# MycroftAI/mycroft-precise

Hardware: AMD Instinct MI355X
Metric: MFCC+GRU windows/sec (node); max concurrent real-time 16 kHz streams (higher is better)
Workload: dtype f32

## Files before the change

### include/precise_engine.h

```cpp
#ifndef PRECISE_ENGINE_H
#define PRECISE_ENGINE_H

#include <stddef.h>
#include <stdint.h>

#ifdef __cplusplus
extern "C" {
#endif

#define PE_ABI_VERSION 8

typedef enum pe_status {
    PE_OK = 0,
    PE_ERR_INVALID = 1,
    PE_ERR_HIP = 2,
    PE_ERR_UNSUPPORTED = 3,
    PE_ERR_NOMEM = 4,
    PE_ERR_EOF = 5
} pe_status;

typedef struct pe_params {
    int32_t sample_rate;
    int32_t window_samples;
    int32_t hop_samples;
// ... 100 lines not shown
int pe_get_info(const pe_engine* e, pe_info* out);

int pe_get_stream_state(pe_engine* e, int32_t* q_out, uint32_t* computed_out, uint32_t* emitted_out);

int pe_set_renumber_at(pe_engine* e, uint32_t call_number);

int pe_set_fused(pe_engine* e, int32_t enabled);

int pe_set_input_projection(pe_engine* e, int32_t enabled);

int pe_set_gru_waves(pe_engine* e, int32_t waves_per_tile);

int pe_set_gru_tiling(pe_engine* e, int32_t tiling);
int pe_get_gru_tiling(const pe_engine* e);

int pe_set_timing(pe_engine* e, int32_t enabled);
int pe_get_last_timing(pe_engine* e, float* mfcc_ms, float* gru_ms);

#ifdef __cplusplus
}
#endif
#endif
```

### mycroft_precise_amd/_lib.py

```python
import ctypes as C
import importlib.util
import os
import weakref

import numpy as np

HERE = os.path.dirname(os.path.abspath(__file__))
LIB_PATH = os.environ.get('PE_LIB') or os.path.join(HERE, 'libprecise_engine.so')

PE_OK, PE_ERR_INVALID, PE_ERR_HIP, PE_ERR_UNSUPPORTED, PE_ERR_NOMEM, PE_ERR_EOF = range(6)
ABI_VERSION = 8


class PeParams(C.Structure):
    _fields_ = [(n, C.c_int32) for n in (
        'sample_rate', 'window_samples', 'hop_samples', 'n_fft', 'n_filt', 'n_mfcc', 'n_features',
        'use_delta', 'mfcc_precision', 'gru_precision', 'vectorizer', 'ring_precision')]


class PeGruLayer(C.Structure):
    _fields_ = [('n_in', C.c_int32), ('units', C.c_int32),
                ('kernel', C.POINTER(C.c_float)), ('recurrent_kernel', C.POINTER(C.c_float)),
                ('bias', C.POINTER(C.c_float))]

# ... 46 lines not shown
                                   C.POINTER(C.c_int64)]),
    'pe_evaluate': (C.c_int, [C.c_void_p, C.c_void_p, C.c_int64, C.c_int32, C.c_void_p, C.c_int64,
                              C.POINTER(C.c_int64)]),
    'pe_set_decoder': (C.c_int, [C.c_void_p, C.c_void_p, C.c_int32, C.c_int32, C.c_int32, C.c_double]),
    'pe_set_trigger': (C.c_int, [C.c_void_p, C.c_int32, C.c_double, C.c_int32]),
    'pe_set_decoder_model': (C.c_int, [C.c_void_p, C.c_int32, C.c_void_p, C.c_int32, C.c_int32, C.c_int32, C.c_double]),
    'pe_set_trigger_model': (C.c_int, [C.c_void_p, C.c_int32, C.c_int32, C.c_double, C.c_int32]),
    'pe_decode_device': (C.c_int, [C.c_void_p, C.c_void_p, C.c_void_p, C.c_void_p, C.c_void_p]),
    'pe_decode': (C.c_int, [C.c_void_p, C.c_void_p, C.c_void_p, C.c_void_p]),
    'pe_get_info': (C.c_int, [C.c_void_p, C.POINTER(PeInfo)]),
    'pe_get_stream_state': (C.c_int, [C.c_void_p, C.c_void_p, C.c_void_p, C.c_void_p]),
    'pe_set_fused': (C.c_int, [C.c_void_p, C.c_int32]),
    'pe_set_gru_waves': (C.c_int, [C.c_void_p, C.c_int32]),
    'pe_set_gru_tiling': (C.c_int, [C.c_void_p, C.c_int32]),
    'pe_get_gru_tiling': (C.c_int, [C.c_void_p]),
    'pe_set_input_projection': (C.c_int, [C.c_void_p, C.c_int32]),
    'pe_set_timing': (C.c_int, [C.c_void_p, C.c_int32]),
    'pe_get_last_timing': (C.c_int, [C.c_void_p, C.POINTER(C.c_float), C.POINTER(C.c_float)]),
}

_lib = None


class HipLibraryMissing(ImportError):
    pass


def _preload_hip_runtime():
    if os.environ.get('PRECISE_AMD_HIP_RUNTIME', '') == 'system':
        return
# ... 305 lines not shown
    def info(self) -> PeInfo:
        i = PeInfo()
        self._check(self._lib.pe_get_info(self._h, C.byref(i)))
        return i

    def stream_state(self):
        q = np.empty(self.n_streams, dtype=np.int32)
        kc = np.empty(self.n_streams, dtype=np.uint32)
        ke = np.empty(self.n_streams, dtype=np.uint32)
        self._check(self._lib.pe_get_stream_state(self._h, q.ctypes.data, kc.ctypes.data, ke.ctypes.data))
        return q, kc, ke

    def set_fused(self, enabled: bool):
        self._check(self._lib.pe_set_fused(self._h, int(bool(enabled))))

    def set_input_projection(self, enabled: bool):
        self._check(self._lib.pe_set_input_projection(self._h, int(bool(enabled))))

    def set_gru_waves(self, waves: int):
        self._check(self._lib.pe_set_gru_waves(self._h, int(waves)))

    def set_gru_tiling(self, tiling: int):
        self._check(self._lib.pe_set_gru_tiling(self._h, int(tiling)))

    def gru_tiling(self) -> int:
        return int(self._lib.pe_get_gru_tiling(self._h))

    def set_timing(self, enabled: bool):
        self._check(self._lib.pe_set_timing(self._h, int(bool(enabled))))

# ... 23 lines not shown
```

### mycroft_precise_amd/csrc/engine.hip

```cpp
#include "../../include/precise_engine.h"
#include "pe_common.h"
#include "gru_cw_pack.h"
#include "mfcc_general_device.h"

#include <algorithm>
#include <cmath>
#include <cstdarg>
#include <cstdio>
#include <cstdlib>
#include <cstring>
#include <string>
#include <vector>

using namespace pe;

namespace {

thread_local std::string g_global_error;

struct DeviceBuf {
    void* p = nullptr;
    size_t bytes = 0;
};

// ... 28 lines not shown
    int64_t device_bytes = 0;
    StreamRec* rec = nullptr;
    int16_t* carry = nullptr;
    const int16_t* kept = nullptr; int kept_chunk = 0;
    const int16_t* call_head = nullptr; int call_head_chunk = 0; bool call_keep = false;
    uint32_t call_no = 1;
    uint32_t renumber_at = 0x7fff0000u;
    bool fused = true;
    int gru_waves = 0;
    bool general = false;
    int row_floats = kRowFloats;
    int carry_cap = kCarryCap;
    GeneralTables gtab{};
    int gru_tiling = -1;
    float* cw_blob = nullptr;
    int n_cus = 256;
    float* ring = nullptr;
    float* proj_ring = nullptr;
    bool proj_ok = false, proj_on = false;
    std::vector<float> proj_w_host, proj_b_host;
    int max_updates = 1;
    uint32_t* ke_hist = nullptr;
    unsigned char* table_blob = nullptr;
    pe_wave::Layout table_layout{};
    float* wxd = nullptr;
    float* wx = nullptr; float* wr1 = nullptr; float* wr2 = nullptr; float* bias = nullptr; float* wd = nullptr;
    bool wide = false;
    float* wide_buf[2][6] = {{nullptr}};
    int wide_kx4[2] = {1, 1};
    float* wide_wd = nullptr;
// ... 735 lines not shown
    for (int m = 0; m < e->n_models; ++m) {
        GruArgs gm = with_model(e, g, m);
        gm.out = g.out + (size_t)m * (size_t)out_stride;
        const int rc = launch_network(e, gm, mode, s, m);
        if (rc) return rc;
    }
    return PE_OK;
}
int launch_networks_many(pe_engine* e, const GruArgs& g, int n_updates, hipStream_t s) {
    if (e->n_models == 1) { PE_HIP(e, launch_gru_many(g, n_updates, e->n_padded, s)); return PE_OK; }
    const ModelSet ms = model_set(e, g);
    PE_HIP(e, launch_gru_many(g, n_updates, e->n_padded, s, &ms, e->n_models));
    return PE_OK;
}

int launch_gru_ring(pe_engine* e, float* out_dev, hipStream_t s, const int32_t* ids = nullptr, int n_active = 0) {
    GruArgs a = gru_args(e);
    a.out = out_dev;
    if (ids) { a.ids = ids; a.n_streams = n_active; }
    return launch_networks(e, a, 1, s, a.n_streams);
}

bool is_pinned(const pe_engine* e, const void* p, size_t bytes) {
    const char* c = static_cast<const char*>(p);
    for (const auto& r : e->pinned)
        if (c >= r.first && c + bytes <= r.first + r.second) return true;
    return false;
}

int async_init(pe_engine* e) {
    if (e->s_compute) return PE_OK;
    PE_HIP(e, hipStreamCreateWithFlags(&e->s_copy, hipStreamNonBlocking));
// ... 86 lines not shown
    }
    if (!keep_call && (rc = flush_kept(e, s))) return rc;
    e->call_head = keep_call ? e->kept : nullptr; e->call_head_chunk = e->kept_chunk; e->call_keep = keep_call;
    struct Reset { pe_engine* e; ~Reset() { e->call_head = nullptr; e->call_head_chunk = 0; e->call_keep = false; } } reset{e};
    e->kept = keep_call ? pcm_dev : nullptr; e->kept_chunk = keep_call ? chunk : 0;
    uint32_t call = 0;
    if ((rc = begin_state_call(e, s, &call))) return rc;
    if (t) { PE_HIP(e, hipEventRecord(e->ev[0], s)); }
    if (raw_out_dev && can_fuse(e, chunk)) {
        GruArgs g = gru_args(e);
        g.call = call;
        g.predict_ke = 1;
        g.chunk = chunk;
        g.out = raw_out_dev;
        if (ids) { g.ids = ids; g.n_streams = n_active; }
        if (e->n_models > 1) {
            const ModelSet ms = model_set(e, g);
            if (e->prm.mfcc_precision == 0) PE_HIP(e, launch_fused_models_f64(mfcc_args<double>(e, pcm_dev, chunk, call, ids, n_active), tables<double>(e), g, ms, e->n_models, e->n_cus, s));
            else PE_HIP(e, launch_fused_models_f32(mfcc_args<float>(e, pcm_dev, chunk, call, ids, n_active), tables<float>(e), g, ms, e->n_models, e->n_cus, s));
        }
        else if (e->prm.mfcc_precision == 0) PE_HIP(e, launch_fused_f64(mfcc_args<double>(e, pcm_dev, chunk, call, ids, n_active), tables<double>(e), g, e->n_cus, s));
        else PE_HIP(e, launch_fused_f32(mfcc_args<float>(e, pcm_dev, chunk, call, ids, n_active), tables<float>(e), g, e->n_cus, s));
        if (t) { PE_HIP(e, hipEventRecord(e->ev[1], s)); PE_HIP(e, hipEventRecord(e->ev[2], s)); e->ev_valid = true; e->ev_has_gru = false; }
    } else {
        if ((rc = launch_mfcc(e, pcm_dev, chunk, s, call, ids, n_active))) return rc;
        if (t) { PE_HIP(e, hipEventRecord(e->ev[1], s)); }
        if (raw_out_dev) {
            if ((rc = launch_gru_ring(e, raw_out_dev, s, ids, n_active))) return rc;
        }
        if (t) { PE_HIP(e, hipEventRecord(e->ev[2], s)); e->ev_valid = true; e->ev_has_gru = raw_out_dev != nullptr; }
    }
    if (feats_out_dev) {
        GatherArgs g{e->n_streams, e->prm.n_features, e->prm.n_mfcc, e->ring_slots, e->prm.ring_precision, e->ring, state_of(e, e->call_no + 1u), feats_out_dev, e->row_floats};
        PE_HIP(e, launch_gather(g, s));
    }
    return PE_OK;
}

}

extern "C" {

int pe_abi_version(void) { return PE_ABI_VERSION; }
// ... 223 lines not shown
    PE_HIP(e, hipSetDevice(e->device));
    PE_DRAIN(e);
    const uint8_t* mask_dev = nullptr;
    if (mask_host) {
        int rc = ensure(e, e->st_mask, (size_t)e->n_streams);
        if (rc) return rc;
        PE_HIP(e, hipMemcpy(e->st_mask.p, mask_host, (size_t)e->n_streams, hipMemcpyHostToDevice));
        mask_dev = static_cast<const uint8_t*>(e->st_mask.p);
    }
    if (mask_dev) { int frc = flush_kept(e, nullptr); if (frc) return frc; }
    else { e->kept = nullptr; e->kept_chunk = 0; }
    uint32_t call = 0;
    { int crc = begin_state_call(e, nullptr, &call); if (crc) return crc; }
    ClearArgs a{e->n_padded, e->ring_slots, mask_dev, state_of(e, call), e->ring, e->prm.ring_precision, e->activation,
                e->proj_on ? e->proj_ring : nullptr,
                e->proj_on ? reinterpret_cast<const float*>(e->table_blob + e->table_layout.proj_b) : nullptr, e->row_floats};
    if (mask_dev) a.n_streams = e->n_streams;
    PE_HIP(e, launch_clear(a, nullptr));
    if (e->n_models > 1 && e->activation)
        PE_HIP(e, launch_clear_activation(mask_dev, e->activation, a.n_streams, e->n_padded, e->n_models - 1, nullptr));
    PE_HIP(e, hipStreamSynchronize(nullptr));
    return PE_OK;
}

int pe_update_device(pe_engine* e, const int16_t* pcm_dev, int32_t chunk, float* raw_out_dev, void* stream) {
    int rc = check_chunk(e, pcm_dev, chunk);
    if (rc) return rc;
    PE_HIP(e, hipSetDevice(e->device));
    PE_DRAIN(e);
    if (!raw_out_dev) return fail(e, PE_ERR_INVALID, "raw_out_dev is null");
    note_user_stream(e, stream);
// ... 190 lines not shown
    PE_HIP(e, hipMemcpy(feats_out_host, e->st_feats.p, feat_bytes, hipMemcpyDeviceToHost));
    return PE_OK;
}

int pe_set_vectors(pe_engine* e, const float* feats_host) {
    if (!e || !feats_host) return fail(e, PE_ERR_INVALID, "null argument to pe_set_vectors");
    PE_HIP(e, hipSetDevice(e->device));
    PE_DRAIN(e);
    int rc;
    if ((rc = pe_clear(e, nullptr))) return rc;
    const size_t feat_bytes = (size_t)e->n_streams * e->prm.n_features * e->prm.n_mfcc * sizeof(float);
    if ((rc = ensure(e, e->st_feats, feat_bytes))) return rc;
    PE_HIP(e, hipMemcpy(e->st_feats.p, feats_host, feat_bytes, hipMemcpyHostToDevice));
    uint32_t call = 0;
    if ((rc = begin_state_call(e, nullptr, &call))) return rc;
    GatherArgs g{e->n_streams, e->prm.n_features, e->prm.n_mfcc, e->ring_slots, e->prm.ring_precision, e->ring, state_of(e, call), static_cast<float*>(e->st_feats.p), e->row_floats};
    PE_HIP(e, launch_scatter(g, nullptr));
    if (e->proj_on)
        PE_HIP(e, launch_project_rows(e->ring, e->proj_ring, reinterpret_cast<const float*>(e->table_blob + e->table_layout.proj_w),
                                      reinterpret_cast<const float*>(e->table_blob + e->table_layout.proj_b), e->prm.n_mfcc,
                                      (long long)e->n_tiles * e->ring_slots * kTileStreams, nullptr));
    PE_HIP(e, hipStreamSynchronize(nullptr));
    return PE_OK;
}

int pe_predict_device(pe_engine* e, const float* feats_dev, int32_t n, float* out_dev, void* stream) {
    if (!e) return PE_ERR_INVALID;
    if (n < 0 || (n > 0 && (!feats_dev || !out_dev))) return fail(e, PE_ERR_INVALID, "bad arguments to pe_predict_device");
    if (n == 0) return PE_OK;
    PE_HIP(e, hipSetDevice(e->device));
    GruArgs a = gru_args(e);
// ... 386 lines not shown

int pe_set_renumber_at(pe_engine* e, uint32_t call_number) {
    if (!e) return PE_ERR_INVALID;
    if (call_number < 8u || call_number > 0x7fff0000u) return fail(e, PE_ERR_INVALID, "renumbering threshold must be in 8..0x7fff0000");
    e->renumber_at = call_number;
    return PE_OK;
}

int pe_set_fused(pe_engine* e, int32_t enabled) {
    if (!e) return PE_ERR_INVALID;
    PE_DRAIN(e);
    e->fused = enabled != 0;
    return PE_OK;
}

int pe_set_input_projection(pe_engine* e, int32_t enabled) {
    if (!e) return PE_ERR_INVALID;
    if (enabled != 0 && enabled != 1) return fail(e, PE_ERR_INVALID, "input projection must be 0 or 1");
    if (enabled && !e->proj_ok) return fail(e, PE_ERR_UNSUPPORTED, "input-projection rows exist for the float32 network of 17..20 units without delta features only");
    if (enabled && e->n_models > 1) return fail(e, PE_ERR_UNSUPPORTED, "input-projection rows are per model: an engine of %d models has none", e->n_models);
    if ((enabled != 0) == e->proj_on) return PE_OK;
    PE_HIP(e, hipSetDevice(e->device));
    PE_DRAIN(e);
    PE_HIP(e, hipDeviceSynchronize());
    e->proj_on = enabled != 0;
    if (e->proj_on && !e->proj_ring) {
        int rc = dev_alloc(e, &e->proj_ring, (size_t)e->n_tiles * e->ring_slots * kTileStreams * kProjRow);
        if (rc) { e->proj_on = false; return rc; }
    }
    return pe_clear(e, nullptr);
// ... 57 lines not shown
```

### mycroft_precise_amd/csrc/kernels.hip

```cpp
#include <cstdlib>
#include <type_traits>
#include "mfcc_device.h"
#include "mfcc_wave_device.h"
#include "gru_device.h"
#include "gru_cw_device.h"
#include "gru_bf16_device.h"
#include "gru_b20_device.h"
#include "gru_x3_device.h"
#include "gru_wide_device.h"
#include "gru_wide_x3_device.h"
#include "mfcc_general_device.h"

namespace pe {

#ifndef PE_FRAME_WPE
#define PE_FRAME_WPE 4
#endif
template <int BYTES>
__device__ __forceinline__ void touch_kernel_arguments() {
    const int* ka = (const int*)__builtin_amdgcn_kernarg_segment_ptr();
    static_assert(BYTES <= 12 * 64, "more lines than this helper requests");
    auto line = [&](int i) -> int { return i * 64 < BYTES ? ka[i * 16] : 0; };
    const int v0 = line(0), v1 = line(1), v2 = line(2), v3 = line(3), v4 = line(4), v5 = line(5), v6 = line(6), v7 = line(7),
              v8 = line(8), v9 = line(9), v10 = line(10), v11 = line(11);
// ... 98 lines not shown
    touch_kernel_arguments<(int)sizeof(GruArgs)>();
    gru_tile<R, MODE, PROJ, KX>(a, blockIdx.x, threadIdx.x);
}

template <int MODE, bool DELTA>
__global__ __launch_bounds__(64) void gru_v_kernel(const GruArgs a) {
    touch_kernel_arguments<(int)sizeof(GruArgs)>();
    gru_tile_v<MODE, DELTA>(a, blockIdx.x, threadIdx.x);
}
__global__ __launch_bounds__(256) void gru_cw_kernel(const GruArgs a) {
    touch_kernel_arguments<(int)sizeof(GruArgs)>();
    extern __shared__ __attribute__((aligned(16))) unsigned char smem[];
    const int wave = __builtin_amdgcn_readfirstlane(threadIdx.x >> 6);
    gru_tile_cw<false>(a, blockIdx.x, wave, threadIdx.x & 63, reinterpret_cast<float*>(smem));
}
static bool cw_four_waves_ok(const GruArgs& a) { return a.ring_slots == kCwSlots && a.n_features <= kCwSlots; }

template <int TPW, int MODE, int WAVES>
__global__ __launch_bounds__(64 * WAVES) void gru_wide_kernel(const WideArgs a) {
    extern __shared__ __attribute__((aligned(16))) unsigned char smem[];
    const int wave = __builtin_amdgcn_readfirstlane(threadIdx.x >> 6);
#ifdef PE_WIDE_STAGGER
    for (int i = (blockIdx.x >> 3) & 31; i > 0; --i) __builtin_amdgcn_s_sleep(PE_WIDE_STAGGER);
#endif
    gru_wide_tile<TPW, MODE, WAVES>(a, blockIdx.x, wave, threadIdx.x & 63, reinterpret_cast<float*>(smem));
}

template <int TPW, int WAVES>
static hipError_t launch_wide_t(const WideArgs& a, int mode, hipStream_t s) {
    const int tiles = (a.base.n_streams + kTileStreams - 1) / kTileStreams;
// ... 160 lines not shown
    } else {
        mfcc_book_tile<R>(m, b - n_gru_blocks - n_frame_blocks);
    }
}
template <class R, class SH, int RG, bool MW, bool PROJ, bool CW = false>
__global__ __launch_bounds__(256) __attribute__((amdgpu_waves_per_eu(PE_FRAME_WPE))) void fused_update_kernel(const MfccStreamArgs<R> m, const WaveTables<R> t, const GruArgs g,
                                                           const int n_gru_blocks, const int n_frame_blocks, const int n_tiles, const int frames_first) {
    fused_update_body<R, SH, RG, MW, PROJ, CW>(m, t, g, n_gru_blocks, n_frame_blocks, n_tiles, frames_first);
}
template <class R, class SH, int RG, bool MW, bool PROJ, bool CW = false>
__global__ __launch_bounds__(256) __attribute__((amdgpu_waves_per_eu(PE_FRAME_WPE))) PE_NO_PK_F32 void fused_update_kernel_nopk(const MfccStreamArgs<R> m, const WaveTables<R> t, const GruArgs g,
                                                           const int n_gru_blocks, const int n_frame_blocks, const int n_tiles, const int frames_first) {
    fused_update_body<R, SH, RG, MW, PROJ, CW>(m, t, g, n_gru_blocks, n_frame_blocks, n_tiles, frames_first);
}

template <class R, class SH, int RG, bool MW, bool CW>
__device__ __forceinline__ void fused_update_models_body(const MfccStreamArgs<R>& m, const WaveTables<R>& t, const GruArgs& g, const ModelSet& ms,
                                                         const int n_gru_blocks, const int n_models, const int n_frame_blocks,
                                                         const int n_tiles, const int frames_first) {
    extern __shared__ __attribute__((aligned(16))) unsigned char smem[];
    touch_kernel_arguments<(int)(sizeof(MfccStreamArgs<R>) + sizeof(WaveTables<R>) + sizeof(GruArgs) + 20)>();
    const int n_net = n_gru_blocks * n_models;
    const int b = role_block(blockIdx.x, n_net, n_frame_blocks, frames_first & kFramesFirst);
    if (b < n_net) {
        const int mi = __builtin_amdgcn_readfirstlane(b / n_gru_blocks);
        const int bl = b - mi * n_gru_blocks;
        const GruArgs gm = model_args(g, ms.net[mi], mi, g.n_streams);
        const int wave = __builtin_amdgcn_readfirstlane(threadIdx.x >> 6);
        __builtin_amdgcn_s_setprio(3);
        int role = wave;
// ... 201 lines not shown
    if (a.row_floats == 2 * kRowFloats) {
        if constexpr (R == 5) {
            if (mode == kRing && a.waves_per_tile == 4) {
                if (mm.ms) PE_NET((NetSmall<R, kRing, false, 2>), (gru_small_kernel<R, kRing, false, 2>), tiles, 64, 0);
                else hipLaunchKernelGGL((gru_mw_kernel<R, false, 2>), dim3(tiles), dim3(256), 0, s, a);
                return hipGetLastError();
            }
        }
        if (mode == kRing) PE_NET((NetSmall<R, kRing, false, 2>), (gru_small_kernel<R, kRing, false, 2>), tiles, 64, 0);
        else if (mode == kRows) PE_NET((NetSmall<R, kRows, false, 2>), (gru_small_kernel<R, kRows, false, 2>), tiles, 64, 0);
        else PE_NET((NetSmall<R, kFeats, false, 2>), (gru_small_kernel<R, kFeats, false, 2>), tiles, 64, 0);
        return hipGetLastError();
    }
    if constexpr (R == 5) {
        if (a.cw) {
            if (mode == kRing && a.waves_per_tile == 4 && cw_four_waves_ok(a)) PE_NET((NetCw), gru_cw_kernel, tiles, 256, kCwLdsBytes);
            else if (a.use_delta) {
                if (mode == kRing) PE_NET((NetV<kRing, true>), (gru_v_kernel<kRing, true>), tiles, 64, 0);
                else if (mode == kRows) PE_NET((NetV<kRows, true>), (gru_v_kernel<kRows, true>), tiles, 64, 0);
                else PE_NET((NetV<kFeats, true>), (gru_v_kernel<kFeats, true>), tiles, 64, 0);
            }
            else if (mode == kRing) PE_NET((NetV<kRing, false>), (gru_v_kernel<kRing, false>), tiles, 64, 0);
            else if (mode == kRows) PE_NET((NetV<kRows, false>), (gru_v_kernel<kRows, false>), tiles, 64, 0);
            else PE_NET((NetV<kFeats, false>), (gru_v_kernel<kFeats, false>), tiles, 64, 0);
            return hipGetLastError();
        }
        if (mode == kRing && a.proj_ring) {
            if (a.waves_per_tile == 4) hipLaunchKernelGGL((gru_mw_kernel<R, true>), dim3(tiles), dim3(256), 0, s, a);
            else hipLaunchKernelGGL((gru_small_kernel<R, kRing, true>), dim3(tiles), dim3(64), 0, s, a);
            return hipGetLastError();
        }
// ... 87 lines not shown
    }
    switch (gru_small_regs(a.units)) {
        case 1: return launch_many_r<1>(a, n_updates, n_padded, s, mm);
        case 2: return launch_many_r<2>(a, n_updates, n_padded, s, mm);
        case 3: return launch_many_r<3>(a, n_updates, n_padded, s, mm);
        case 4: return launch_many_r<4>(a, n_updates, n_padded, s, mm);
        case 5: return launch_many_r<5>(a, n_updates, n_padded, s, mm);
        case 6: return launch_many_r<6>(a, n_updates, n_padded, s, mm);
        case 7: return launch_many_r<7>(a, n_updates, n_padded, s, mm);
        case 8: return launch_many_r<8>(a, n_updates, n_padded, s, mm);
        default: return hipErrorInvalidValue;
    }
}

static bool fused_models_four_waves(int n_models, int tiles, int n_cus) { return (long long)n_models * tiles <= 2LL * n_cus; }

template <class R, int RG>
static hipError_t launch_fused_rg(const MfccStreamArgs<R>& m, const WaveTables<R>& t, const GruArgs& g, int n_cus, hipStream_t s,
                                  const ModelSet* ms = nullptr, int n_models = 1) {
    const int tiles = (m.geo.n_streams + kTileStreams - 1) / kTileStreams;
    const size_t lds = frame_lds(t);
    const bool by_simd = g.cw && g.waves_per_tile == 4 && cw_four_waves_ok(g) && tiles <= n_cus;
    const int frames_first = ((g.waves_per_tile != 4 && tiles >= 4 * n_cus) ? 1 : 0) | (by_simd ? kBySimd : 0);
    const int fb = stream_frame_blocks(m.geo.n_streams, n_cus, tiles <= n_cus ? 2 : (frames_first & kFramesFirst) ? 3 : 4);
    const int gru_blocks = g.waves_per_tile == 4 ? tiles : (tiles + 3) / 4;
    const int fb_ = fb, book = tiles;
    const dim3 grid(gru_blocks + fb_ + book);
    if (ms) {
        if (g.proj_ring) return hipErrorInvalidValue;
        const dim3 mgrid(gru_blocks * n_models + fb_ + book);
// ... 3 lines not shown
                    PE_LAUNCH_R(R, fused_update_models_kernel, (ShapeStock, RG, true, true), mgrid, dim3(256), lds > kCwLdsBytes ? lds : kCwLdsBytes, s, m, t, g, gru_blocks, n_models, fb_, tiles, frames_first, *ms);
                } else {
                    const int gb = (tiles + 3) / 4;
                    PE_LAUNCH_R(R, fused_update_models_kernel, (ShapeStock, RG, false, true), dim3(gb * n_models + fb_ + book), dim3(256), lds, s, m, t, g, gb, n_models, fb_, tiles, frames_first & ~kBySimd, *ms);
                }
                return hipGetLastError();
            }
        }
        if (g.waves_per_tile == 4) PE_LAUNCH_R(R, fused_update_models_kernel, (ShapeStock, RG, true, false), mgrid, dim3(256), lds, s, m, t, g, gru_blocks, n_models, fb_, tiles, frames_first, *ms);
        else if constexpr (RG <= 5) PE_LAUNCH_R(R, fused_update_models_kernel, (ShapeStock, RG, false, false), mgrid, dim3(256), lds, s, m, t, g, gru_blocks, n_models, fb_, tiles, frames_first, *ms);
        else return hipErrorInvalidValue;
        return hipGetLastError();
    }
    if constexpr (RG == 5) {
        if (g.cw) {
            if (g.waves_per_tile == 4 && cw_four_waves_ok(g)) {
                PE_LAUNCH_R(R, fused_update_kernel, (ShapeStock, RG, true, false, true), grid, dim3(256), lds > kCwLdsBytes ? lds : kCwLdsBytes, s, m, t, g, gru_blocks, fb_, tiles, frames_first);
            } else {
                const int gb = (tiles + 3) / 4;
                PE_LAUNCH_R(R, fused_update_kernel, (ShapeStock, RG, false, false, true), dim3(gb + fb_ + book), dim3(256), lds, s, m, t, g, gb, fb_, tiles, frames_first);
            }
            return hipGetLastError();
        }
    }
    if constexpr (RG == 5) {
        if (g.proj_ring) {
            if (g.waves_per_tile == 4) PE_LAUNCH_R(R, fused_update_kernel, (ShapeStock, RG, true, true), grid, dim3(256), lds, s, m, t, g, gru_blocks, fb_, tiles, frames_first);
            else PE_LAUNCH_R(R, fused_update_kernel, (ShapeStock, RG, false, true), grid, dim3(256), lds, s, m, t, g, gru_blocks, fb_, tiles, frames_first);
            return hipGetLastError();
        }
// ... 166 lines not shown
    const int RF = a.row_floats;
    const long long total = (long long)a.n_streams * a.n_features * RF;
    if (idx >= total) return;
    const int f = (int)(idx % RF);
    const int t = (int)((idx / RF) % a.n_features);
    const long long s = idx / ((long long)RF * a.n_features);
    const long long tile = s / kTileStreams;
    const int j = (int)(s % kTileStreams);
    const float v = f < a.n_mfcc ? a.out[(s * a.n_features + t) * a.n_mfcc + f] : 0.0f;
    const size_t at = (((size_t)tile * a.ring_slots + t) * kTileStreams + j) * RF + f;
    if (a.ring_bf16) reinterpret_cast<__bf16*>(const_cast<float*>(a.ring))[at] = (__bf16)v;
    else const_cast<float*>(a.ring)[at] = v;
    if (f == 0 && t == 0) {
        a.st.rec[rec_at(a.st.n_padded, s, 0)] = StreamRec{0, (uint32_t)a.n_features, (uint32_t)a.n_features, a.st.call};
        a.st.rec[rec_at(a.st.n_padded, s, 1)] = StreamRec{0, (uint32_t)a.n_features, (uint32_t)a.n_features, a.st.call - 1u};
    }
}

hipError_t launch_scatter(const GatherArgs& a, hipStream_t s) {
    const long long total = (long long)a.n_streams * a.n_features * a.row_floats;
    if (total == 0) return hipSuccess;
    hipLaunchKernelGGL(scatter_kernel, dim3((unsigned)((total + 255) / 256)), dim3(256), 0, s, a);
    return hipGetLastError();
}

__global__ void renumber_kernel(const StreamState st, const int n_padded) {
    const int s = blockIdx.x * blockDim.x + threadIdx.x;
    if (s >= n_padded) return;
    const RecPair both = rec_request(st.rec, st.n_padded, s);
    const int side = rec_side(both, st.call);
// ... 16 lines not shown
}

hipError_t launch_renumber(const StreamState& st, int n_padded, hipStream_t s) {
    hipLaunchKernelGGL(renumber_kernel, dim3((n_padded + 255) / 256), dim3(256), 0, s, st, n_padded);
    return hipGetLastError();
}

__global__ void clear_kernel(const ClearArgs a) {
    const long long s = blockIdx.x;
    if (s >= a.n_streams) return;
    if (a.mask && !a.mask[s]) return;
    if (threadIdx.x == 0) {
        a.st.rec[rec_at(a.st.n_padded, s, 0)] = StreamRec{0, 0u, 0u, a.st.call};
        a.st.rec[rec_at(a.st.n_padded, s, 1)] = StreamRec{0, 0u, 0u, a.st.call - 1u};
        if (a.activation) a.activation[s] = 0;
    }
    const long long tile = s / kTileStreams;
    const int j = (int)(s % kTileStreams);
    for (int i = threadIdx.x; i < a.ring_slots * a.row_floats; i += blockDim.x) {
        const int slot = i / a.row_floats, f = i % a.row_floats;
        const size_t at = (((size_t)tile * a.ring_slots + slot) * kTileStreams + j) * a.row_floats + f;
        if (a.ring_bf16) reinterpret_cast<__bf16*>(a.ring)[at] = (__bf16)0.0f;
        else a.ring[at] = 0.0f;
    }
    if (a.proj_ring)
        for (int i = threadIdx.x; i < a.ring_slots * kProjRow; i += blockDim.x) {
            const int slot = i / kProjRow, o = i % kProjRow;
            a.proj_ring[((size_t)tile * a.ring_slots + slot) * kTileStreams * kProjRow + (size_t)((o >> 2) & 3) * (kTileStreams * 16) + j * 16 + (o >> 4) * 4 + (o & 3)] = a.proj_b[o];
        }
}
// ... 130 lines not shown
```

### mycroft_precise_amd/csrc/pe_common.h

```cpp
#pragma once
#include <hip/hip_runtime.h>
#include <stdint.h>
#include "mfcc_wave_tables.h"

namespace pe {

constexpr int kTileStreams = 16;
constexpr int kRowFloats = 16;
constexpr int kCarryCap = 512;
constexpr int kNfft = 512;
constexpr int kBins = kNfft / 2 + 1;
constexpr int kMaxFilt = 64;
constexpr int kCwSlots = 32;

template <class R> struct cplx { R x, y; };

constexpr int kMaxFrameRows = 4096;
constexpr int kFrameWaves = 4;

template <class R>
struct WaveTables {
    const void* blob;
    pe_wave::Layout L;
};
// ... 17 lines not shown
        return (uint32_t)(((uint64_t)x * mul) >> 32) >> shift;
#endif
    }
};

struct __attribute__((aligned(16))) StreamRec { int32_t q; uint32_t kc, ke, wcall; };

__host__ __device__ __forceinline__ size_t rec_at(const uint32_t, const long long s, const int side) { return 2 * (size_t)s + (size_t)side; }

struct StreamState {
    StreamRec* rec;
    int16_t* carry;
    uint32_t n_padded;
    uint32_t call;
};

struct RecPair { StreamRec r0, r1; };
__device__ __forceinline__ RecPair rec_request(const StreamRec* rec, const uint32_t n_padded, const long long s) {
    RecPair p;
    p.r0 = rec[rec_at(n_padded, s, 0)];
    p.r1 = rec[rec_at(n_padded, s, 1)];
    return p;
}
__device__ __forceinline__ int rec_side(const RecPair& p, const uint32_t call) {
    return (call - p.r1.wcall) - 1u < (call - p.r0.wcall) - 1u ? 1 : 0;
}
__device__ __forceinline__ StreamRec rec_pick(const RecPair& p, const int side) {
    StreamRec r;
    r.q = side ? p.r1.q : p.r0.q; r.kc = side ? p.r1.kc : p.r0.kc; r.ke = side ? p.r1.ke : p.r0.ke; r.wcall = side ? p.r1.wcall : p.r0.wcall;
    return r;
// ... 64 lines not shown
    const float* wx;
    const float* wxd;
    int use_delta;
    const float* wr1;
    const float* wr2;
    const float* bias;
    const float* wd;
    float dense_bias;
    const float* cw;
    int bf16;
    const void* wx_bf16;
    const void* wr_bf16;
    const float* wd_bf16;
    const void* b20;
    const void* x3;
    const void* reserved_;
    const int32_t* ids;
    const StreamRec* rec;
    uint32_t n_padded, call;
    const uint32_t* ke_plain;
    const float* ring;
    int ring_bf16;
    const float* proj_ring;
    int ring_slots;
    int predict_ke;
    int chunk, window, hop, frame_len;
    const float* feats;
    int row_stride;
    float* out;
    int row_floats;
    int waves_per_tile;
// ... 60 lines not shown

struct WideArgs {
    GruArgs base;
    WideLayerArgs layer[2];
    int n_layers;
    int units;
    const float* wd;
};

struct GatherArgs {
    int n_streams, n_features, n_mfcc, ring_slots, ring_bf16;
    const float* ring;
    StreamState st;
    float* out;
    int row_floats = kRowFloats;
};

struct ClearArgs {
    int n_streams, ring_slots;
    const uint8_t* mask;
    StreamState st;
    float* ring;
    int ring_bf16;
    int32_t* activation;
    float* proj_ring;
    const float* proj_b;
    int row_floats = kRowFloats;
};

struct DecodeArgs {
    int n_streams;
    const float* raw;
    const double* cd;
    int cd_len, min_out, out_range;
    double center;
    double* conf_out;
    int32_t* activation;
    unsigned char* fired_out;
    double threshold;
    int trigger_level, rearm;
};
hipError_t launch_decode(const DecodeArgs& a, hipStream_t s);
// ... 29 lines not shown
```

Measured before the change: 271.3 million.

## Reuse per-window GRU hidden states across sliding windows instead of full recompute

Adds a persistent per-stream store of GRU hidden states, one for each window start offset, plus a marker of how far each stream has advanced. When only one or two new frames arrive, each stored chain is advanced by those frames instead of rerunning the full T-step recurrence for every window, and the chains are spread across waves. A full recompute path fills the store when a stream is cold. The feature is on by default, and the store is reset by clear and scatter. It costs extra device memory and global stores each call, and only matches the windowed-reset GRU semantics when the chain bookkeeping is exact.

```diff
diff --git a/include/precise_engine.h b/include/precise_engine.h
--- a/include/precise_engine.h
+++ b/include/precise_engine.h
@@ -138,6 +138,9 @@
 int pe_set_gru_tiling(pe_engine* e, int32_t tiling);
 int pe_get_gru_tiling(const pe_engine* e);
 
+int pe_set_window_states(pe_engine* e, int32_t enabled);
+int pe_get_window_states(const pe_engine* e);
+
 int pe_set_timing(pe_engine* e, int32_t enabled);
 int pe_get_last_timing(pe_engine* e, float* mfcc_ms, float* gru_ms);
 
diff --git a/mycroft_precise_amd/_lib.py b/mycroft_precise_amd/_lib.py
--- a/mycroft_precise_amd/_lib.py
+++ b/mycroft_precise_amd/_lib.py
@@ -84,6 +84,8 @@
     'pe_set_gru_waves': (C.c_int, [C.c_void_p, C.c_int32]),
     'pe_set_gru_tiling': (C.c_int, [C.c_void_p, C.c_int32]),
     'pe_get_gru_tiling': (C.c_int, [C.c_void_p]),
+    'pe_set_window_states': (C.c_int, [C.c_void_p, C.c_int32]),
+    'pe_get_window_states': (C.c_int, [C.c_void_p]),
     'pe_set_input_projection': (C.c_int, [C.c_void_p, C.c_int32]),
     'pe_set_timing': (C.c_int, [C.c_void_p, C.c_int32]),
     'pe_get_last_timing': (C.c_int, [C.c_void_p, C.POINTER(C.c_float), C.POINTER(C.c_float)]),
@@ -419,6 +421,12 @@
     def set_fused(self, enabled: bool):
         self._check(self._lib.pe_set_fused(self._h, int(bool(enabled))))
 
+    def set_window_states(self, enabled: bool):
+        self._check(self._lib.pe_set_window_states(self._h, int(bool(enabled))))
+
+    def get_window_states(self) -> bool:
+        return self._lib.pe_get_window_states(self._h) == 1
+
     def set_input_projection(self, enabled: bool):
         self._check(self._lib.pe_set_input_projection(self._h, int(bool(enabled))))
 
diff --git a/mycroft_precise_amd/csrc/engine.hip b/mycroft_precise_amd/csrc/engine.hip
--- a/mycroft_precise_amd/csrc/engine.hip
+++ b/mycroft_precise_amd/csrc/engine.hip
@@ -66,6 +66,8 @@
     GeneralTables gtab{};
     int gru_tiling = -1;
     float* cw_blob = nullptr;
+    void* win = nullptr;
+    bool win_on = true;
     int n_cus = 256;
     float* ring = nullptr;
     float* proj_ring = nullptr;
@@ -831,8 +833,28 @@
     return PE_OK;
 }
 
-int launch_gru_ring(pe_engine* e, float* out_dev, hipStream_t s, const int32_t* ids = nullptr, int n_active = 0) {
+bool win_engine_ok(const pe_engine* e) {
+    return e->cw_blob && !e->general && !e->wide && e->n_models == 1 && !e->prm.use_delta && e->prm.gru_precision == 0
+        && e->row_floats == kRowFloats && e->table_layout.mel_pad == 10 && e->prm.n_features <= kWinMaxFeatures;
+}
+bool win_call_ok(pe_engine* e, const GruArgs& g, int chunk) {
+    if (!e->win_on || !win_engine_ok(e)) return false;
+    if (!g.cw || g.waves_per_tile != 4 || e->ring_slots != kWinSlots) return false;
+    if (chunk > emit_window(e->prm) - frame_len_of(e->prm)) return false;
+    if (!e->win) {
+        const size_t bytes = win_bytes((uint32_t)e->n_padded);
+        unsigned char* p = nullptr;
+        if (dev_alloc(e, &p, bytes)) return false;
+        if (hipMemset(p, 0, bytes) != hipSuccess) { dev_free(e, p, bytes); return false; }
+        e->win = p;
+    }
+    return true;
+}
+WinMark* win_marks_of(const pe_engine* e) { return e->win ? win_marks(e->win, (uint32_t)e->n_padded) : nullptr; }
+
+int launch_gru_ring(pe_engine* e, float* out_dev, hipStream_t s, const int32_t* ids = nullptr, int n_active = 0, int slide_chunk = 0) {
     GruArgs a = gru_args(e);
+    if (slide_chunk > 0 && win_call_ok(e, a, slide_chunk)) a.win = e->win;
     a.out = out_dev;
     if (ids) { a.ids = ids; a.n_streams = n_active; }
     return launch_networks(e, a, 1, s, a.n_streams);
@@ -949,6 +971,7 @@
         g.chunk = chunk;
         g.out = raw_out_dev;
         if (ids) { g.ids = ids; g.n_streams = n_active; }
+        if (win_call_ok(e, g, chunk)) g.win = e->win;
         if (e->n_models > 1) {
             const ModelSet ms = model_set(e, g);
             if (e->prm.mfcc_precision == 0) PE_HIP(e, launch_fused_models_f64(mfcc_args<double>(e, pcm_dev, chunk, call, ids, n_active), tables<double>(e), g, ms, e->n_models, e->n_cus, s));
@@ -961,7 +984,7 @@
         if ((rc = launch_mfcc(e, pcm_dev, chunk, s, call, ids, n_active))) return rc;
         if (t) { PE_HIP(e, hipEventRecord(e->ev[1], s)); }
         if (raw_out_dev) {
-            if ((rc = launch_gru_ring(e, raw_out_dev, s, ids, n_active))) return rc;
+            if ((rc = launch_gru_ring(e, raw_out_dev, s, ids, n_active, chunk))) return rc;
         }
         if (t) { PE_HIP(e, hipEventRecord(e->ev[2], s)); e->ev_valid = true; e->ev_has_gru = raw_out_dev != nullptr; }
     }
@@ -1215,7 +1238,8 @@
     { int crc = begin_state_call(e, nullptr, &call); if (crc) return crc; }
     ClearArgs a{e->n_padded, e->ring_slots, mask_dev, state_of(e, call), e->ring, e->prm.ring_precision, e->activation,
                 e->proj_on ? e->proj_ring : nullptr,
-                e->proj_on ? reinterpret_cast<const float*>(e->table_blob + e->table_layout.proj_b) : nullptr, e->row_floats};
+                e->proj_on ? reinterpret_cast<const float*>(e->table_blob + e->table_layout.proj_b) : nullptr, e->row_floats,
+                win_marks_of(e)};
     if (mask_dev) a.n_streams = e->n_streams;
     PE_HIP(e, launch_clear(a, nullptr));
     if (e->n_models > 1 && e->activation)
@@ -1436,7 +1460,8 @@
     PE_HIP(e, hipMemcpy(e->st_feats.p, feats_host, feat_bytes, hipMemcpyHostToDevice));
     uint32_t call = 0;
     if ((rc = begin_state_call(e, nullptr, &call))) return rc;
-    GatherArgs g{e->n_streams, e->prm.n_features, e->prm.n_mfcc, e->ring_slots, e->prm.ring_precision, e->ring, state_of(e, call), static_cast<float*>(e->st_feats.p), e->row_floats};
+    GatherArgs g{e->n_streams, e->prm.n_features, e->prm.n_mfcc, e->ring_slots, e->prm.ring_precision, e->ring, state_of(e, call), static_cast<float*>(e->st_feats.p), e->row_floats,
+                 win_marks_of(e)};
     PE_HIP(e, launch_scatter(g, nullptr));
     if (e->proj_on)
         PE_HIP(e, launch_project_rows(e->ring, e->proj_ring, reinterpret_cast<const float*>(e->table_blob + e->table_layout.proj_w),
@@ -1853,6 +1878,19 @@
     return PE_OK;
 }
 
+int pe_set_window_states(pe_engine* e, int32_t enabled) {
+    if (!e) return PE_ERR_INVALID;
+    if (enabled != 0 && enabled != 1) return fail(e, PE_ERR_INVALID, "window states must be 0 or 1");
+    PE_DRAIN(e);
+    e->win_on = enabled != 0;
+    return PE_OK;
+}
+
+int pe_get_window_states(const pe_engine* e) {
+    if (!e) return -2;
+    return e->win_on && win_engine_ok(e) ? 1 : 0;
+}
+
 int pe_set_input_projection(pe_engine* e, int32_t enabled) {
     if (!e) return PE_ERR_INVALID;
     if (enabled != 0 && enabled != 1) return fail(e, PE_ERR_INVALID, "input projection must be 0 or 1");
diff --git a/mycroft_precise_amd/csrc/gru_slide_device.h b/mycroft_precise_amd/csrc/gru_slide_device.h
--- /dev/null
+++ b/mycroft_precise_amd/csrc/gru_slide_device.h
@@ -0,0 +1,170 @@
+#pragma once
+#include "gru_cw_device.h"
+
+namespace pe {
+
+__device__ __forceinline__ void win_load(const float* slot, const int lane, float (&h)[5]) {
+    const f32x4 v = *reinterpret_cast<const f32x4*>(slot + 4 * lane);
+    h[4] = slot[256 + lane];
+    h[0] = v[0]; h[1] = v[1]; h[2] = v[2]; h[3] = v[3];
+}
+__device__ __forceinline__ void win_store(float* slot, const int lane, const float (&h)[5], const int tune) {
+    const f32x4 v = {h[0], h[1], h[2], h[3]};
+    if (tune & 1) return;
+    if (tune & 2) {
+        *reinterpret_cast<f32x4*>(slot + 4 * lane) = v;
+        slot[256 + lane] = h[4];
+        return;
+    }
+    asm volatile("global_store_dwordx4 %0, %1, off sc1\n\ts_nop 1" :: "v"(slot + 4 * lane), "v"(v) : "memory");
+    __hip_atomic_store(slot + 256 + lane, h[4], __ATOMIC_RELAXED, __HIP_MEMORY_SCOPE_AGENT);
+}
+
+template <int WAVES>
+__device__ __forceinline__ int slide_owner(const int c) {
+    if (WAVES == 1 || c < 3) return 0;
+    const int i = c - 3;
+    return i < 2 * (WAVES - 1) ? 1 + i % (WAVES - 1) : (i - 2 * (WAVES - 1)) % WAVES;
+}
+
+template <int WAVES>
+__device__ __forceinline__ void gru_tile_slide(const GruArgs& a, const int tile, const int wave, const int lane) {
+    const int g = lane >> 4, j = lane & 15;
+    const long long stream = (long long)tile * kTileStreams + j;
+    const bool valid = stream < a.n_streams;
+    const int T = a.n_features;
+    const float* cw = a.cw;
+    const long long sid = gru_stream_of(a, stream, valid);
+    const KeRequest ke_req = gru_ke_request(a, sid);
+    WinMark* const marks = win_marks(a.win, a.n_padded);
+    const WinMark mk = marks[sid];
+    CwStep<false> S;
+    S.load(cw, lane);
+    float wx[4][4], wd[5];
+    f32x4 bias[4];
+#pragma unroll
+    for (int tl = 0; tl < 4; ++tl)
+#pragma unroll
+        for (int kk = 0; kk < 4; ++kk) {
+            wx[tl][kk] = cw[CwPack::WX + (tl * 4 + kk) * 64 + lane];
+            bias[tl][kk] = cw[CwPack::BIAS + (tl * 4 + kk) * 64 + lane];
+        }
+#pragma unroll
+    for (int rho = 0; rho < 5; ++rho) wd[rho] = wave == 0 ? a.wd[rho * 64 + lane] : 0.f;
+    const float* const xbase = a.ring + gru_ring_cell(a, sid) * kRowFloats + 4 * g;
+    float* const hbase = reinterpret_cast<float*>(a.win) + (size_t)(sid >> 4) * kWinSlots * kWinSlotFloats;
+    const int hl = 16 * g + (int)(sid & 15);
+    const int tune = a.row_stride;
+    auto x_row = [&](const uint32_t frame) -> f32x4 {
+        return *reinterpret_cast<const f32x4*>(xbase + (size_t)(frame & (uint32_t)(kWinSlots - 1)) * kTileStreams * kRowFloats);
+    };
+    auto h_at = [&](const uint32_t start) -> float* { return hbase + (size_t)(start & (uint32_t)(kWinSlots - 1)) * kWinSlotFloats; };
+
+    const uint32_t e_new = gru_ke_resolve(a, ke_req);
+    const uint32_t n = e_new - mk.upto;
+    const bool current = !valid || (mk.valid != 0u && n <= 2u);
+    const bool slide = __builtin_amdgcn_ballot_w64(current) == ~0ull;
+    const bool one = __builtin_amdgcn_ballot_w64(valid && n >= 1u) != 0ull;
+    const bool two = __builtin_amdgcn_ballot_w64(valid && n >= 2u) != 0ull;
+    const int last = !slide ? -1 : two ? T + 1 : one ? T : 0;
+    auto next_chain = [&](int c) -> int {
+        for (++c; c <= last && slide_owner<WAVES>(c) != wave; ++c) {}
+        return c;
+    };
+    const f32x4 x0 = x_row(mk.upto), x1 = x_row(mk.upto + 1u);
+    float h[5] = {0.f, 0.f, 0.f, 0.f, 0.f};
+    int c = next_chain(-1);
+    if (c <= last) win_load(h_at(mk.upto - (uint32_t)T + (uint32_t)c), hl, h);
+    __syncthreads();
+
+    if (slide) {
+        const uint32_t f0 = mk.upto, k0 = mk.upto - (uint32_t)T;
+        f32x4 i0[4], i1[4];
+#pragma unroll
+        for (int tl = 0; tl < 4; ++tl) { i0[tl] = f32x4{0.f, 0.f, 0.f, 0.f}; i1[tl] = i0[tl]; }
+        if (one) {
+            const f32x4 x0 = x_row(f0), x1 = x_row(f0 + 1u);
+#pragma unroll
+            for (int tl = 0; tl < 4; ++tl) i0[tl] = cw_xproj(wx[tl], bias[tl], x0);
+            if (two) {
+#pragma unroll
+                for (int tl = 0; tl < 4; ++tl) i1[tl] = cw_xproj(wx[tl], bias[tl], x1);
+            }
+        }
+        S.pin();
+        const int last = two ? T + 1 : one ? T : 0;
+        auto next_chain = [&](int c) -> int {
+            for (++c; c <= last && slide_owner<WAVES>(c) != wave; ++c) {}
+            return c;
+        };
+        auto request = [&](const int c, float (&h)[5]) {
+            const float* const p = h_at(k0 + (uint32_t)c);
+#pragma unroll
+            for (int rho = 0; rho < 5; ++rho) h[rho] = p[rho * 64];
+        };
+        float hout[5], h[5], hn[5];
+#pragma unroll
+        for (int rho = 0; rho < 5; ++rho) hout[rho] = hn[rho] = 0.f;
+        int c = next_chain(-1);
+        if (c <= last) request(c, h);
+        bool head_due = wave == 0;
+        while (c <= last) {
+            const int cn = next_chain(c);
+            if (cn <= last) request(cn, hn);
+            if (c >= 1 && c <= T) {
+                float hs[5];
+#pragma unroll
+                for (int rho = 0; rho < 5; ++rho) hs[rho] = c == T ? 0.f : h[rho];
+                S.step(hs, i0[kTZ], i0[kTX], i0[kTC], i0[kTV]);
+#pragma unroll
+                for (int rho = 0; rho < 5; ++rho) h[rho] = n >= 1u ? hs[rho] : h[rho];
+            }
+            if (two && c >= 2) {
+                float hs[5];
+#pragma unroll
+                for (int rho = 0; rho < 5; ++rho) hs[rho] = c == T + 1 ? 0.f : h[rho];
+                S.step(hs, i1[kTZ], i1[kTX], i1[kTC], i1[kTV]);
+#pragma unroll
+                for (int rho = 0; rho < 5; ++rho) h[rho] = n >= 2u ? hs[rho] : h[rho];
+            }
+            if (c >= 1 && valid) win_store(h_at(k0 + (uint32_t)c), hl, h, tune);
+            if (wave == 0 && c <= 2) {
+#pragma unroll
+                for (int rho = 0; rho < 5; ++rho) hout[rho] = n == (uint32_t)c ? h[rho] : hout[rho];
+            }
+            if (head_due && (cn > 2 || cn > last)) {
+                cw_head(a, hout, wd, stream, valid, g);
+                head_due = false;
+            }
+#pragma unroll
+            for (int rho = 0; rho < 5; ++rho) h[rho] = hn[rho];
+            c = cn;
+        }
+    } else {
+        const uint32_t k0 = e_new - (uint32_t)T;
+        for (int i = 0; i < T; ++i) {
+            const int r = i % (2 * WAVES);
+            if (r != wave && r != 2 * WAVES - 1 - wave) continue;
+            float h[5];
+#pragma unroll
+            for (int rho = 0; rho < 5; ++rho) h[rho] = 0.f;
+            f32x4 x = x_row(k0 + (uint32_t)i);
+            for (int t = i; t < T; ++t) {
+                const f32x4 xn = x_row(k0 + (uint32_t)(t + 1 < T ? t + 1 : t));
+                const f32x4 aZ = cw_xproj(wx[kTZ], bias[kTZ], x), aX = cw_xproj(wx[kTX], bias[kTX], x);
+                const f32x4 aC = cw_xproj(wx[kTC], bias[kTC], x), aV = cw_xproj(wx[kTV], bias[kTV], x);
+                S.step(h, aZ, aX, aC, aV);
+                x = xn;
+            }
+            if (valid) {
+                float* const p = h_at(k0 + (uint32_t)i);
+#pragma unroll
+                for (int rho = 0; rho < 5; ++rho) p[rho * 64] = h[rho];
+            }
+            if (i == 0) cw_head(a, h, wd, stream, valid, g);
+        }
+    }
+    if (wave == 0 && valid && g == 0) marks[sid] = WinMark{e_new, 1u};
+}
+
+}
diff --git a/mycroft_precise_amd/csrc/kernels.hip b/mycroft_precise_amd/csrc/kernels.hip
--- a/mycroft_precise_amd/csrc/kernels.hip
+++ b/mycroft_precise_amd/csrc/kernels.hip
@@ -4,6 +4,7 @@
 #include "mfcc_wave_device.h"
 #include "gru_device.h"
 #include "gru_cw_device.h"
+#include "gru_slide_device.h"
 #include "gru_bf16_device.h"
 #include "gru_b20_device.h"
 #include "gru_x3_device.h"
@@ -136,6 +137,14 @@
     const int wave = __builtin_amdgcn_readfirstlane(threadIdx.x >> 6);
     gru_tile_cw<false>(a, blockIdx.x, wave, threadIdx.x & 63, reinterpret_cast<float*>(smem));
 }
+template <int WAVES>
+__global__ __launch_bounds__(64 * WAVES) void gru_slide_kernel(const GruArgs a) {
+    touch_kernel_arguments<(int)sizeof(GruArgs)>();
+    const int wave = __builtin_amdgcn_readfirstlane(threadIdx.x >> 6);
+    gru_tile_slide<WAVES>(a, blockIdx.x, wave, threadIdx.x & 63);
+}
+constexpr int kSlideWaves = 4;
+static bool slide_ok(const GruArgs& a) { return a.win && a.cw && !a.use_delta && a.ring_slots == kWinSlots && a.n_features <= kWinMaxFeatures; }
 static bool cw_four_waves_ok(const GruArgs& a) { return a.ring_slots == kCwSlots && a.n_features <= kCwSlots; }
 
 template <int TPW, int MODE, int WAVES>
@@ -326,6 +335,33 @@
     fused_update_body<R, SH, RG, MW, PROJ, CW>(m, t, g, n_gru_blocks, n_frame_blocks, n_tiles, frames_first);
 }
 
+template <class R, class SH>
+__device__ __forceinline__ void fused_slide_body(const MfccStreamArgs<R>& m, const WaveTables<R>& t, const GruArgs& g,
+                                                 const int n_gru_blocks, const int n_frame_blocks, const int frames_first) {
+    extern __shared__ __attribute__((aligned(16))) unsigned char smem[];
+    touch_kernel_arguments<(int)(sizeof(MfccStreamArgs<R>) + sizeof(WaveTables<R>) + sizeof(GruArgs) + 12)>();
+    const int b = role_block(blockIdx.x, n_gru_blocks, n_frame_blocks, frames_first & kFramesFirst);
+    if (b < n_gru_blocks) {
+        const int wave = __builtin_amdgcn_readfirstlane(threadIdx.x >> 6);
+        if (!(frames_first & 16)) __builtin_amdgcn_s_setprio(3);
+        gru_tile_slide<4>(g, b, wave, threadIdx.x & 63);
+    } else if (b < n_gru_blocks + n_frame_blocks) {
+        mfcc_frame_tasks<R, SH, true, true>(m, t, smem, (b - n_gru_blocks) * kFrameWaves, n_frame_blocks * kFrameWaves, false);
+    } else {
+        mfcc_book_tile<R>(m, b - n_gru_blocks - n_frame_blocks);
+    }
+}
+template <class R, class SH>
+__global__ __launch_bounds__(256) __attribute__((amdgpu_waves_per_eu(PE_FRAME_WPE))) void fused_slide_kernel(const MfccStreamArgs<R> m, const WaveTables<R> t, const GruArgs g,
+                                                          const int n_gru_blocks, const int n_frame_blocks, const int frames_first) {
+    fused_slide_body<R, SH>(m, t, g, n_gru_blocks, n_frame_blocks, frames_first);
+}
+template <class R, class SH>
+__global__ __launch_bounds__(256) __attribute__((amdgpu_waves_per_eu(PE_FRAME_WPE))) PE_NO_PK_F32 void fused_slide_kernel_nopk(const MfccStreamArgs<R> m, const WaveTables<R> t, const GruArgs g,
+                                                          const int n_gru_blocks, const int n_frame_blocks, const int frames_first) {
+    fused_slide_body<R, SH>(m, t, g, n_gru_blocks, n_frame_blocks, frames_first);
+}
+
 template <class R, class SH, int RG, bool MW, bool CW>
 __device__ __forceinline__ void fused_update_models_body(const MfccStreamArgs<R>& m, const WaveTables<R>& t, const GruArgs& g, const ModelSet& ms,
                                                          const int n_gru_blocks, const int n_models, const int n_frame_blocks,
@@ -557,7 +593,11 @@
     }
     if constexpr (R == 5) {
         if (a.cw) {
-            if (mode == kRing && a.waves_per_tile == 4 && cw_four_waves_ok(a)) PE_NET((NetCw), gru_cw_kernel, tiles, 256, kCwLdsBytes);
+            if (mode == kRing && a.win) {
+                if (mm.ms || !slide_ok(a)) return hipErrorInvalidValue;
+                hipLaunchKernelGGL((gru_slide_kernel<kSlideWaves>), dim3(tiles), dim3(64 * kSlideWaves), 0, s, a);
+            }
+            else if (mode == kRing && a.waves_per_tile == 4 && cw_four_waves_ok(a)) PE_NET((NetCw), gru_cw_kernel, tiles, 256, kCwLdsBytes);
             else if (a.use_delta) {
                 if (mode == kRing) PE_NET((NetV<kRing, true>), (gru_v_kernel<kRing, true>), tiles, 64, 0);
                 else if (mode == kRows) PE_NET((NetV<kRows, true>), (gru_v_kernel<kRows, true>), tiles, 64, 0);
@@ -675,6 +715,16 @@
 }
 
 static bool fused_models_four_waves(int n_models, int tiles, int n_cus) { return (long long)n_models * tiles <= 2LL * n_cus; }
+
+static int slide_tune_flags() {
+    static const int f = std::getenv("PE_TUNE_SLIDE_FLAGS") ? std::atoi(std::getenv("PE_TUNE_SLIDE_FLAGS")) : 0;
+    return f;
+}
+static int slide_frame_per_cu(int tiles, int n_cus) {
+    static const int forced = std::getenv("PE_TUNE_SLIDE_FB") ? std::atoi(std::getenv("PE_TUNE_SLIDE_FB")) : 0;
+    if (forced) return forced;
+    return tiles <= n_cus ? 2 : 4;
+}
 
 template <class R, int RG>
 static hipError_t launch_fused_rg(const MfccStreamArgs<R>& m, const WaveTables<R>& t, const GruArgs& g, int n_cus, hipStream_t s,
@@ -708,6 +758,12 @@
     }
     if constexpr (RG == 5) {
         if (g.cw) {
+            if (g.win) {
+                if (!slide_ok(g)) return hipErrorInvalidValue;
+                const int sfb = stream_frame_blocks(m.geo.n_streams, n_cus, slide_frame_per_cu(tiles, n_cus));
+                PE_LAUNCH_R(R, fused_slide_kernel, (ShapeStock), dim3(tiles + sfb + book), dim3(256), lds, s, m, t, g, tiles, sfb, slide_tune_flags());
+                return hipGetLastError();
+            }
             if (g.waves_per_tile == 4 && cw_four_waves_ok(g)) {
                 PE_LAUNCH_R(R, fused_update_kernel, (ShapeStock, RG, true, false, true), grid, dim3(256), lds > kCwLdsBytes ? lds : kCwLdsBytes, s, m, t, g, gru_blocks, fb_, tiles, frames_first);
             } else {
@@ -904,6 +960,7 @@
     if (f == 0 && t == 0) {
         a.st.rec[rec_at(a.st.n_padded, s, 0)] = StreamRec{0, (uint32_t)a.n_features, (uint32_t)a.n_features, a.st.call};
         a.st.rec[rec_at(a.st.n_padded, s, 1)] = StreamRec{0, (uint32_t)a.n_features, (uint32_t)a.n_features, a.st.call - 1u};
+        if (a.win_marks) a.win_marks[s] = WinMark{0u, 0u};
     }
 }
 
@@ -950,6 +1007,7 @@
         a.st.rec[rec_at(a.st.n_padded, s, 0)] = StreamRec{0, 0u, 0u, a.st.call};
         a.st.rec[rec_at(a.st.n_padded, s, 1)] = StreamRec{0, 0u, 0u, a.st.call - 1u};
         if (a.activation) a.activation[s] = 0;
+        if (a.win_marks) a.win_marks[s] = WinMark{0u, 0u};
     }
     const long long tile = s / kTileStreams;
     const int j = (int)(s % kTileStreams);
diff --git a/mycroft_precise_amd/csrc/pe_common.h b/mycroft_precise_amd/csrc/pe_common.h
--- a/mycroft_precise_amd/csrc/pe_common.h
+++ b/mycroft_precise_amd/csrc/pe_common.h
@@ -55,6 +55,16 @@
     uint32_t n_padded;
     uint32_t call;
 };
+
+constexpr int kWinSlots = 32;
+constexpr int kWinMaxFeatures = 29;
+constexpr int kWinSlotFloats = 5 * 64;
+struct __attribute__((aligned(8))) WinMark { uint32_t upto, valid; };
+__host__ __device__ __forceinline__ size_t win_state_floats(const uint32_t n_padded) { return (size_t)(n_padded / 16u) * kWinSlots * kWinSlotFloats; }
+__host__ __device__ __forceinline__ size_t win_bytes(const uint32_t n_padded) { return win_state_floats(n_padded) * sizeof(float) + (size_t)n_padded * sizeof(WinMark); }
+__host__ __device__ __forceinline__ WinMark* win_marks(void* win, const uint32_t n_padded) {
+    return reinterpret_cast<WinMark*>(static_cast<float*>(win) + win_state_floats(n_padded));
+}
 
 struct RecPair { StreamRec r0, r1; };
 __device__ __forceinline__ RecPair rec_request(const StreamRec* rec, const uint32_t n_padded, const long long s) {
@@ -149,7 +159,7 @@
     const float* wd_bf16;
     const void* b20;
     const void* x3;
-    const void* reserved_;
+    void* win;
     const int32_t* ids;
     const StreamRec* rec;
     uint32_t n_padded, call;
@@ -240,6 +250,7 @@
     StreamState st;
     float* out;
     int row_floats = kRowFloats;
+    WinMark* win_marks = nullptr;
 };
 
 struct ClearArgs {
@@ -252,6 +263,7 @@
     float* proj_ring;
     const float* proj_b;
     int row_floats = kRowFloats;
+    WinMark* win_marks = nullptr;
 };
 
 struct DecodeArgs {
```

Result: no change. 270.2 million (-0.4%).
